# soon-yau/upgpt

Hardware: AMD Instinct MI355X
Metric: 256x256 images/sec, 50-step DDIM, bs=8/GPU; UNet MFMA util % (higher is better)
Workload: dtype f16; 1 GPU; BASELINE configs[1]: bs=8/GPU, 256x256 px (latent 4x32x32), 50-step DDIM eta=0, text-only cond [B,87,768], UNet(bbox.yaml) + VAE decode, EMA weights, no CFG; batch_per_gpu=8, ddim_steps=50, batches_in_flight_per_gpu=4, lane_hw_queues=measured, parallelism=replica-dp1, one all-gather of images per batch

## Files before the change

include/upk.h:

```cpp
#ifndef UPK_H_
#define UPK_H_

#include <stddef.h>
#include <stdint.h>

#ifdef __cplusplus
extern "C" {
#endif

#define UPK_VERSION 100

#define UPK_OK 0
#define UPK_EINVAL (-1)
#define UPK_ESHAPE (-2)
#define UPK_EWORKSPACE (-3)
#define UPK_EHIP (-4)
#define UPK_ENODEV (-5)

typedef struct upk_ctx upk_ctx;
typedef void* upk_stream;

int upk_version(void);
int upk_create(upk_ctx** out, int device);
int upk_destroy(upk_ctx* ctx);
const char* upk_last_error(upk_ctx* ctx);
int upk_set_workspace(upk_ctx* ctx, void* dptr, size_t bytes);
int upk_num_cus(upk_ctx* ctx);

int upk_pack_weight_f16(upk_ctx* ctx, const float* w_oihw, int cout, int cin, int kh, int kw,
                        const int32_t* row_map, int n_rows_packed, const int32_t* col_map,
                        int cin_packed, void* w_packed, upk_stream stream);
size_t upk_packed_weight_bytes(int n_rows_packed, int cin_packed, int kh, int kw);

#define UPK_F_SILU 0x1
#define UPK_F_GEGLU 0x2
#define UPK_F_OUT_F32 0x4
#define UPK_F_OUT_NCHW_F32 0x8
// ... 35 lines not shown
  const void* x4;
  int32_t c3, c4;
  int32_t ld3, ld4;
  const float* gno_gamma;
  const float* gno_beta;
  void* gno_y;
  float gno_eps;
  int32_t gno_silu, gno_ld, gno_skip_y;
  float* ln_rows_out;
  const float* ln_rows_in;
  int32_t ln_rows_slots;
  const void* w_phase;
  int32_t gn_stats_cap;
  const void* pf_next;
  int64_t pf_bytes;
} upk_conv_desc;

int upk_conv2d_nhwc_f16(upk_ctx* ctx, const upk_conv_desc* d, upk_stream stream);

int upk_conv_gn_fused(upk_ctx* ctx, const upk_conv_desc* d, int* mode, int* nblk);
int upk_groupnorm_finalize_f32(upk_ctx* ctx, const float* partials, int nblk, int ld, int batch, int hw, int c,
                               int groups, float* ws, upk_stream stream);
int upk_conv_ln_rows(upk_ctx* ctx, const upk_conv_desc* d, int* slots);

typedef struct upk_mlp_desc {
  const void* x;
  int32_t ldx, m, c, inner;
  const void* w1;
  const float* b1;
  const float* u1;
  float ln_eps;
  int32_t ln_dim;
  const void* w2;
  const float* b2;
  int32_t n_out, n_pad;
  const void* residual;
  int32_t ld_res;
  void* y;
// ... 189 lines not shown
```

upgpt_amd/_lib.py:

```python
import contextlib
import ctypes as C
import os
import threading

import torch
from ._check import require

_HERE = os.path.dirname(os.path.abspath(__file__))
LIB_PATH = os.environ.get("UPK_LIB") or os.path.join(_HERE, "libupk.so")

SYMBOLS = [
    "upk_version", "upk_create", "upk_destroy", "upk_last_error", "upk_set_workspace", "upk_num_cus",
    "upk_pack_weight_f16", "upk_packed_weight_bytes", "upk_conv2d_nhwc_f16", "upk_gemm_f16",
    "upk_conv_autotune", "upk_conv_override", "upk_conv_num_configs", "upk_conv_config_name", "upk_conv_gn_fused",
    "upk_conv_ln_rows",
    "upk_geglu_mlp_f16", "upk_geglu_mlp_supported", "upk_cross_block_f16", "upk_cross_block_supported", "upk_head_block_f16", "upk_head_block_supported",
    "upk_attention_f16", "upk_groupnorm_nhwc_f16", "upk_groupnorm_stats_nhwc_f16", "upk_groupnorm_chunks", "upk_groupnorm_apply_nhwc_f16", "upk_groupnorm_finalize_f32", "upk_groupnorm_ws_bytes",
    "upk_layernorm_f16", "upk_timestep_embed_f16",
    "upk_nchw_f32_to_nhwc_f16", "upk_nhwc_f16_to_nchw_f32", "upk_f32_to_f16", "upk_ddim_step_f32",
    "upk_ddim_step_cfg_f32", "upk_ddim_step_edit_f32", "upk_plms_step_f32", "upk_ddpm_step_f32", "upk_attention_causal_f16", "upk_attention_qproj_f16", "upk_embed_tokens_f16",
    "upk_patchify_nchw_f32_f16", "upk_vit_assemble_f16", "upk_gather_rows_f16",
    "upk_image_finish_u8", "upk_ssim_ws_bytes", "upk_ssim_u8",
    "upk_lpips_input_f16", "upk_relu_pool_nhwc_f16", "upk_lpips_ws_bytes", "upk_lpips_layer_f16",
    "upk_advance_step", "upk_step_autoadvance", "upk_kernel_launches", "upk_graph_begin", "upk_graph_end", "upk_graph_launch", "upk_graph_destroy",
    "upk_prof_enable", "upk_prof_collect",
    "upk_stream_create_cumask", "upk_stream_destroy", "upk_probe_placement", "upk_probe_clock",
]

F_SILU, F_GEGLU, F_OUT_F32, F_OUT_NCHW_F32, F_UPSAMPLE2X, F_PAD_ASYM = 0x1, 0x2, 0x4, 0x8, 0x10, 0x20
DDPM_X0, DDPM_CLIP = 0x1, 0x2
# ... 22 lines not shown
        ("bias", C.c_void_p), ("residual", C.c_void_p), ("ld_res", C.c_int32),
        ("rowvec", C.c_void_p), ("rv_batch_stride", C.c_int32), ("rv_step_stride", C.c_int32),
        ("step", C.c_void_p), ("y", C.c_void_p), ("ldy", C.c_int32),
        ("vt", C.c_void_p), ("vt_from", C.c_int32), ("vt_heads", C.c_int32), ("vt_dhead", C.c_int32),
        ("vt_ld", C.c_int32), ("vt_tokens", C.c_int32), ("flags", C.c_int32),
        ("tune_cfg", C.c_int32), ("tune_splitk", C.c_int32),
        ("ln_colsum", C.c_void_p), ("ln_eps", C.c_float), ("ln_dim", C.c_int32),
        ("gn_stats_ws", C.c_void_p), ("gn_groups", C.c_int32),
        ("x3", C.c_void_p), ("x4", C.c_void_p),
        ("c3", C.c_int32), ("c4", C.c_int32), ("ld3", C.c_int32), ("ld4", C.c_int32),
        ("gno_gamma", C.c_void_p), ("gno_beta", C.c_void_p), ("gno_y", C.c_void_p), ("gno_eps", C.c_float),
        ("gno_silu", C.c_int32), ("gno_ld", C.c_int32), ("gno_skip_y", C.c_int32),
        ("ln_rows_out", C.c_void_p), ("ln_rows_in", C.c_void_p), ("ln_rows_slots", C.c_int32),
        ("w_phase", C.c_void_p), ("gn_stats_cap", C.c_int32),
        ("pf_next", C.c_void_p), ("pf_bytes", C.c_int64),
    ]


class MlpDesc(C.Structure):
    _fields_ = [
        ("x", C.c_void_p), ("ldx", C.c_int32), ("m", C.c_int32), ("c", C.c_int32), ("inner", C.c_int32),
        ("w1", C.c_void_p), ("b1", C.c_void_p), ("u1", C.c_void_p), ("ln_eps", C.c_float), ("ln_dim", C.c_int32),
        ("w2", C.c_void_p), ("b2", C.c_void_p), ("n_out", C.c_int32), ("n_pad", C.c_int32),
        ("residual", C.c_void_p), ("ld_res", C.c_int32), ("y", C.c_void_p), ("ldy", C.c_int32),
        ("gn_stats_ws", C.c_void_p), ("hw", C.c_int32), ("rows_per_wg", C.c_int32),
    ]


class XblockDesc(C.Structure):
    _fields_ = [
        ("a1", C.c_void_p), ("lda", C.c_int32), ("m", C.c_int32), ("c", C.c_int32), ("heads", C.c_int32), ("d", C.c_int32),
# ... 23 lines not shown

def load_library(path=None):
    global _lib
    with _lib_lock:
        if _lib is not None and path is None:
            return _lib
        p = path or LIB_PATH
        if not os.path.exists(p):
            raise RuntimeError(
                "libupk.so not found at %s: build it with `python -m upgpt_amd.build` "
                "(hipcc --offload-arch=gfx950). There is no CPU fallback." % p)
        lib = C.CDLL(p)
        vp, i32, i64, f32 = C.c_void_p, C.c_int, C.c_longlong, C.c_float
        protos = {
            "upk_version": (C.c_int, []),
            "upk_create": (C.c_int, [C.POINTER(vp), i32]),
            "upk_destroy": (C.c_int, [vp]),
            "upk_last_error": (C.c_char_p, [vp]),
            "upk_set_workspace": (C.c_int, [vp, vp, C.c_size_t]),
            "upk_num_cus": (C.c_int, [vp]),
            "upk_pack_weight_f16": (C.c_int, [vp, vp, i32, i32, i32, i32, vp, i32, vp, i32, vp, vp]),
            "upk_packed_weight_bytes": (C.c_size_t, [i32, i32, i32, i32]),
            "upk_conv2d_nhwc_f16": (C.c_int, [vp, C.POINTER(ConvDesc), vp]),
            "upk_gemm_f16": (C.c_int, [vp, vp, i32, i32, i32, vp, i32, i32, vp, vp, i32, vp, i32, i32, vp]),
            "upk_conv_autotune": (C.c_int, [vp, C.POINTER(ConvDesc), vp, i32, C.POINTER(C.c_int), C.POINTER(C.c_int),
                                            C.POINTER(C.c_float), C.POINTER(C.c_float)]),
            "upk_conv_override": (C.c_int, [vp, i32, i32]),
            "upk_conv_num_configs": (C.c_int, []),
            "upk_conv_config_name": (C.c_char_p, [i32]),
            "upk_conv_ln_rows": (C.c_int, [vp, C.POINTER(ConvDesc), C.POINTER(C.c_int)]),
# ... 8 lines not shown
            "upk_attention_causal_f16": (C.c_int, [vp, vp, i32, i64, vp, i32, i64, vp, i32, vp, i32, i64,
                                                   i32, i32, i32, i32, f32, vp]),
            "upk_attention_qproj_f16": (C.c_int, [vp, vp, i32, i64, i32, i32, f32, vp, vp, vp, vp, i32, i64, vp, i32, vp,
                                                  i32, i64, i32, i32, i32, i32, i32, f32, vp]),
            "upk_embed_tokens_f16": (C.c_int, [vp, vp, vp, vp, i32, i32, i32, i32, vp, i32, vp]),
            "upk_gather_rows_f16": (C.c_int, [vp, vp, i32, vp, i32, i32, i32, vp, i32, vp]),
            "upk_patchify_nchw_f32_f16": (C.c_int, [vp, vp, i32, i32, i32, i32, i32, vp, i32, vp]),
            "upk_vit_assemble_f16": (C.c_int, [vp, vp, i32, vp, vp, i32, i32, i32, vp, i32, vp]),
            "upk_groupnorm_nhwc_f16": (C.c_int, [vp, vp, i32, i32, vp, i32, i32, i32, i32, i32, vp, vp,
                                                 f32, i32, vp, i32, vp, vp]),
            "upk_groupnorm_stats_nhwc_f16": (C.c_int, [vp, vp, i32, i32, vp, i32, i32, i32, i32, i32, vp, vp]),
            "upk_groupnorm_chunks": (C.c_int, [i32]),
            "upk_groupnorm_apply_nhwc_f16": (C.c_int, [vp, vp, i32, i32, vp, i32, i32, i32, i32, i32, vp, vp,
                                                       f32, i32, vp, i32, vp, i32, i32, i32, vp, i32, i32, vp]),
            "upk_conv_gn_fused": (C.c_int, [vp, C.POINTER(ConvDesc), C.POINTER(C.c_int), C.POINTER(C.c_int)]),
            "upk_groupnorm_finalize_f32": (C.c_int, [vp, vp, i32, i32, i32, i32, i32, i32, vp, vp]),
            "upk_groupnorm_ws_bytes": (C.c_size_t, [i32, i32]),
            "upk_layernorm_f16": (C.c_int, [vp, vp, i32, i32, i32, vp, vp, f32, vp, i32, vp]),
            "upk_timestep_embed_f16": (C.c_int, [vp, vp, i32, i32, f32, vp, i32, vp]),
            "upk_nchw_f32_to_nhwc_f16": (C.c_int, [vp, vp, i32, i32, i32, vp, i32, i32, i32, f32, vp]),
            "upk_nhwc_f16_to_nchw_f32": (C.c_int, [vp, vp, i32, i32, i32, i32, vp, vp]),
            "upk_f32_to_f16": (C.c_int, [vp, vp, i32, i32, vp, i32, vp]),
            "upk_ddim_step_f32": (C.c_int, [vp, vp, vp, vp, vp, vp, vp, vp, i32, i32, i32, i32, vp]),
            "upk_ddim_step_cfg_f32": (C.c_int, [vp, vp, vp, vp, vp, vp, vp, vp, i32, i32, i32, i32, f32, vp]),
            "upk_ddim_step_edit_f32": (C.c_int, [vp, vp, vp, vp, vp, vp, vp, i32, vp, vp, vp, vp, i32, i32, i32, i32, f32,
                                                 i32, vp]),
            "upk_plms_step_f32": (C.c_int, [vp, vp, vp, vp, vp, vp, vp, vp, i32, i32, i32, i32, f32, i32, vp]),
            "upk_ddpm_step_f32": (C.c_int, [vp, vp, vp, vp, vp, vp, vp, vp, vp, vp, vp, i32, i32, i32, i32, i32, vp]),
            "upk_image_finish_u8": (C.c_int, [vp, vp, i32, i32, i32, i32, i64, i32, i32, i32, i32, vp, i64, i32, i64, i32,
                                              C.POINTER(C.c_float), vp]),
# ... 10 lines not shown
            "upk_graph_end": (C.c_int, [vp, vp, C.POINTER(vp)]),
            "upk_graph_launch": (C.c_int, [vp, vp, vp]),
            "upk_graph_destroy": (C.c_int, [vp, vp]),
            "upk_prof_enable": (C.c_int, [vp, i32]),
            "upk_prof_collect": (C.c_int, [vp, C.POINTER(C.c_double), C.POINTER(C.c_longlong)]),
            "upk_stream_create_cumask": (C.c_int, [vp, C.POINTER(C.c_uint32), i32, C.POINTER(vp)]),
            "upk_stream_destroy": (C.c_int, [vp, vp]),
            "upk_probe_placement": (C.c_int, [vp, vp, i32, i32, vp]),
            "upk_probe_clock": (C.c_int, [vp, vp, i64, vp]),
        }
        require(sorted(protos) == sorted(SYMBOLS), "ctypes prototypes and SYMBOLS differ", RuntimeError)
        for name, (res, args) in protos.items():
            fn = getattr(lib, name)
            fn.restype = res
            fn.argtypes = args
        if path is None:
            _lib = lib
        return lib


def _ptr(t):
    if t is None:
        return None
    if isinstance(t, int):
        return t
    return t.data_ptr()


class Context:

# ... 61 lines not shown
        self._chk(self.lib.upk_embed_tokens_f16(self.h, _ptr(ids), _ptr(tok), _ptr(pos), rows, seq, dim, vocab, _ptr(out),
                                                ld, self._s()))

    def gather_rows(self, x, ldx, idx, n, n_src, dim, y, ldy):
        self._chk(self.lib.upk_gather_rows_f16(self.h, _ptr(x), ldx, _ptr(idx), n, n_src, dim, _ptr(y), ldy, self._s()))

    def groupnorm(self, x1, c1, ld1, x2, c2, ld2, batch, hw, groups, gamma, beta, eps, silu, y, ldy, ws):
        self._chk(self.lib.upk_groupnorm_nhwc_f16(self.h, _ptr(x1), c1, ld1, _ptr(x2), c2, ld2, batch, hw, groups,
                                                  _ptr(gamma), _ptr(beta), eps, int(silu), _ptr(y), ldy, _ptr(ws),
                                                  self._s()))

    def conv_gn_fused(self, desc):
        f, n = C.c_int(0), C.c_int(0)
        self._chk(self.lib.upk_conv_gn_fused(self.h, C.byref(desc), C.byref(f), C.byref(n)))
        return f.value, n.value

    def gn_stats_floats(self, batch, n_pad, cap=32):
        return batch * max(32, cap) * 2 * max(n_pad, 32)

    def groupnorm_ws_bytes(self, batch, hw):
        return self.lib.upk_groupnorm_ws_bytes(batch, hw)

    def layernorm(self, x, ldx, rows, d, gamma, beta, eps, y, ldy):
        self._chk(self.lib.upk_layernorm_f16(self.h, _ptr(x), ldx, rows, d, _ptr(gamma), _ptr(beta), eps,
                                             _ptr(y), ldy, self._s()))

    def timestep_embed(self, t, n, dim, max_period, out, ld_out):
        self._chk(self.lib.upk_timestep_embed_f16(self.h, _ptr(t), n, dim, max_period, _ptr(out), ld_out, self._s()))

    def nchw_to_nhwc(self, x, batch, c, hw, y, ldy, c_off=0, zero_pad_to=0, scale=1.0):
# ... 205 lines not shown
```

upgpt_amd/csrc/igemm.hip:

```cpp
#include "igemm_common.h"

namespace {
using namespace upkd;


template <int MI, int NI, int WM, int WN, int KS>
__global__ __launch_bounds__(WM* WN * 64) void igemm_kernel(const IgemmArgs a) {
  constexpr int BM = MI * 16 * WM;
  constexpr int BN = NI * 16 * WN;
  constexpr int NT = WM * WN * 64;
  constexpr int A_IT = (BM * 4 + NT - 1) / NT;
  constexpr int B_IT = (BN * 4 + NT - 1) / NT;
  constexpr int A_TILE = BM * 32;
  constexpr int B_TILE = BN * 32;
  constexpr int A_STAGE = KS * A_TILE;
  constexpr int B_STAGE = KS * B_TILE;

  __shared__ __attribute__((aligned(16))) f16 smem[2 * (A_STAGE + B_STAGE)];
  f16* sA = smem;
  f16* sB = smem + 2 * A_STAGE;

  const int tid = threadIdx.x;
  const int lane = tid & 63;
  const int wave = tid >> 6;
// ... 178 lines not shown
    return;
  }
  if (a.partial) {
    slab_t* slab = (slab_t*)a.partial + ((long)zs * (a.ph_on ? 4 : 1) + ph) * a.M * a.npad;
#pragma unroll
    for (int i = 0; i < MI; ++i) {
      const int m = mw + i * 16 + lc;
      if (m >= a.M) continue;
      const unsigned roff = (unsigned)m * (unsigned)a.npad;
#pragma unroll
      for (int j = 0; j < NI; ++j) {
        const int n = nw + j * 16 + lg * 4;
        if (n < a.npad && !ABL_ON(ABL_NOSLAB)) slab_store(slab + roff + n, acc[i][j]);
      }
    }
    return;
  }
  if (a.lnr_in) Epi::lnr_fix<MI, NI>(a, mw, nw, lc, lg, acc);
  Epi::tile<MI, NI, WM, WN>(a, m0, mw, nw, lc, lg, acc, wm, wn, (float*)smem, a.M);
}


template <int P>
__device__ __forceinline__ void wait_vmcnt() {
  asm volatile("s_waitcnt vmcnt(%0)" ::"n"(P) : "memory");
}

template <int MI, int NI, int WM, int WN, int KS, int NBUF, bool APP = false, bool LNF = false, int LW = 4>
__global__ __launch_bounds__(256 + LW * 64) void igemm_ws_kernel(const IgemmArgs a) {
  static_assert(WM * WN == 4 || WM * WN == 1, "4 consumer waves");
// ... 343 lines not shown
    if ABL_ON(ABL_NOEPI) return;
    auto frag_sum = [&](int f) {
      f32x4 v = *(const f32x4*)(red + ((0 * NF + f) * 64 + lane) * 4);
#pragma unroll
      for (int w = 1; w < 4; ++w) v += *(const f32x4*)(red + ((w * NF + f) * 64 + lane) * 4);
      return v;
    };
    slab_t* slab = a.partial ? (slab_t*)a.partial + ((long)zs * (a.ph_on ? 4 : 1) + ph) * a.M * a.npad : nullptr;
    if (slab) {
      for (int f = wave; f < NF; f += EW) {
        const int i = f / NI, j = f - i * NI;
        const int m = m0 + i * 16 + lc;
        const int n = n0 + j * 16 + lg * 4;
        if (n < a.npad && m < a.M && !ABL_ON(ABL_NOSLAB)) slab_store(slab + (unsigned)m * (unsigned)a.npad + n, frag_sum(f));
      }
      return;
    }
    constexpr int FW = (NF + EW - 1) / EW;
    if (Epi::plain(a)) {
      const Epi::Plain P(a);
      Epi::Plain::Row rows[FW];
      f32x4 bvs[FW], rvs[FW];
      f16x4 rrs[FW];
#pragma unroll
      for (int q = 0; q < FW; ++q) {
        const int f = wave + EW * q;
        const int i = f / NI, j = f - i * NI;
        const int n = n0 + j * 16 + lg * 4;
        rows[q] = P.row(a, f < NF ? m0 + i * 16 + lc : a.M, a.M);
        bvs[q] = P.bias4(a, n);
// ... 147 lines not shown
    return;
  }
  if (a.partial) {
    slab_t* slab = (slab_t*)a.partial + ((long)zs * (a.ph_on ? 4 : 1) + ph) * a.M * a.npad;
#pragma unroll
    for (int i = 0; i < MI; ++i) {
      const int m = mw + i * 16 + lc;
      if (m >= a.M) continue;
      const unsigned roff = (unsigned)m * (unsigned)a.npad;
#pragma unroll
      for (int j = 0; j < NI; ++j) {
        const int n = nw + j * 16 + lg * 4;
        if (n < a.npad && !ABL_ON(ABL_NOSLAB)) slab_store(slab + roff + n, acc[i][j]);
      }
    }
    return;
  }
  if constexpr (SHARE) {
    if (Epi::plain(a) && !a.lnr_out) {
      float* hand = (float*)((char*)smem + HAND_OFF) + wave * (MI * NJ1) * 256;
      f32x4 acc1[MI][NJ0];
#pragma unroll
      for (int i = 0; i < MI; ++i)
#pragma unroll
        for (int j = 0; j < NI; ++j) {
          if (j < NJ0) acc1[i][j] = acc[i][j];
          else *(f32x4*)(hand + ((i * NJ1 + (j - NJ0)) * 64 + lane) * 4) = acc[i][j];
        }
      asm volatile("s_waitcnt lgkmcnt(0)" ::: "memory");
      __builtin_amdgcn_s_barrier();
// ... 13 lines not shown
  if (wave == 0) {
    asm volatile("s_waitcnt vmcnt(0)" ::: "memory");
    STAMP(4);
  }
#endif
#undef STAMP
}

__global__ __launch_bounds__(256) void igemm_reduce_kernel(const IgemmArgs a, int splitk) {
  const int nq = a.npad >> 2;
  const long idx = (long)blockIdx.x * 256 + threadIdx.x;
  const long total = (long)a.M * nq;
  if (idx >= total) return;
  const int m = (int)(idx / nq);
  const int n = (int)(idx - (long)m * nq) * 4;
  const long slab = (long)a.M * a.npad * (a.ph_on ? 4 : 1);
  const slab_t* p = (const slab_t*)a.partial + ((long)ph_id(a) * a.M + m) * a.npad + n;
  f32x4 v = {0, 0, 0, 0}, g = {0, 0, 0, 0};
  const f32x4 z4 = {0.f, 0.f, 0.f, 0.f};
  if (a.flags & UPK_F_GEGLU) {
    if (n & 32) return;
    for (int z = 0; z < splitk; ++z) {
      v += slab_load4(p + z * slab);
      g += slab_load4(p + z * slab + 32);
    }
  } else {
    for (int z0 = 0; z0 < splitk; z0 += 4) {
      f32x4 t[4];
#pragma unroll
      for (int u = 0; u < 4; ++u) t[u] = z0 + u < splitk ? slab_load4(p + (long)(z0 + u) * slab) : z4;
#pragma unroll
      for (int u = 0; u < 4; ++u) v += t[u];
    }
  }
  IgemmArgs b = a;
  b.partial = nullptr;
  const RowCtx rc = Epi::row(b, m, b.M);
  Epi::store(b, rc, n, v, g, Epi::bias4(b, n), Epi::bias4(b, (a.flags & UPK_F_GEGLU) ? n + 32 : a.npad),
             Epi::fetch(b, rc, n));
}

struct GnApply {
  const float* gamma;
  const float* beta;
  f16* yn;
  float eps;
  int ldn, silu, skip_y, cpg, hw;
};

template <int V>
struct VecIO {
  static __device__ __forceinline__ void ldf(const float* p, bool on, float (&o)[V]) {
    if constexpr (V == 4) {
      const f32x4 w = on ? *(const f32x4*)p : (f32x4){0.f, 0.f, 0.f, 0.f};
// ... 308 lines not shown
extern "C" int upk_conv_num_configs(void) { return kNumCfgs + astat_num_configs() + bt_num_configs(); }
extern "C" const char* upk_conv_config_name(int cfg) {
  if (cfg >= kNumCfgs + astat_num_configs()) return bt_config_name(cfg - kNumCfgs - astat_num_configs());
  if (cfg >= kNumCfgs) return astat_config_name(cfg - kNumCfgs);
  return (cfg >= 0 && cfg < kNumCfgs) ? kCfgs[cfg].name : "?";
}
extern "C" int upk_conv_override(upk_ctx* ctx, int cfg, int splitk) {
  if (!ctx) return UPK_EINVAL;
  if (cfg >= upk_conv_num_configs()) return upk_fail(ctx, UPK_EINVAL, "conv_override: configuration %d of %d", cfg, upk_conv_num_configs());
  ctx->cfg_override = cfg;
  ctx->splitk_override = splitk;
  return UPK_OK;
}

static int conv_impl(upk_ctx* ctx, const upk_conv_desc* d, upk_stream stream_, bool launch, int* gn_fused,
                     int* gn_nblk = nullptr, int* lnr_slots = nullptr) {
  if (lnr_slots) *lnr_slots = 0;
  if (!ctx || !d) return UPK_EINVAL;
  hipStream_t stream = (hipStream_t)stream_;
  if (!d->x1 || !d->w_packed || !d->y) return upk_fail(ctx, UPK_EINVAL, "conv: null x1/w/y");
  if (d->c1 <= 0 || (d->c1 & 31) || (d->c2 & 31) || d->c2 < 0)
    return upk_fail(ctx, UPK_ESHAPE, "conv: channels must be multiples of 32 (c1=%d c2=%d)", d->c1, d->c2);
  if (d->c2 > 0 && !d->x2) return upk_fail(ctx, UPK_EINVAL, "conv: c2>0 but x2 null");
  if (d->ksize != 1 && d->ksize != 3) return upk_fail(ctx, UPK_ESHAPE, "conv: ksize %d", d->ksize);
  if (d->stride != 1 && d->stride != 2) return upk_fail(ctx, UPK_ESHAPE, "conv: stride %d", d->stride);
  if ((d->ld1 & 7) || (d->c2 && (d->ld2 & 7)) || (d->n_pad & 15) || d->n_pad <= 0)
    return upk_fail(ctx, UPK_EINVAL, "conv: leading dims must be multiples of 8, n_pad of 16");
  const int flags = d->flags;
  const bool geglu = flags & UPK_F_GEGLU;
  if (geglu && (d->n_pad & 63)) return upk_fail(ctx, UPK_ESHAPE, "conv: GEGLU needs n_pad %% 64 == 0");
  if (!(flags & UPK_F_OUT_NCHW_F32) && (d->ldy & 3)) return upk_fail(ctx, UPK_EINVAL, "conv: ldy %% 4");
  if (d->residual && (d->ld_res & 3)) return upk_fail(ctx, UPK_EINVAL, "conv: ld_res %% 4");
// ... 133 lines not shown
    best = want_cfg;
    best_sk = sk;
  }
  const bool is_as = want_cfg >= kNumCfgs && !is_bt;
  if (is_as) {
    if (!astat_plan(ctx, a, want_cfg - kNumCfgs, want_sk, &aspl) || (want_sk > 1 && want_sk > aspl.npass))
      return upk_fail(ctx, UPK_ESHAPE, "conv: A-stationary configuration %s (passes per workgroup %d) does not fit this launch",
                      astat_config_name(want_cfg - kNumCfgs), want_sk);
    best = want_cfg;
    best_sk = 1;
  }
  for (int c = 0; c < kNumCfgs && !is_as && !is_bt; ++c) {
    if (want_cfg >= 0 && c != want_cfg) continue;
    if (a.ln_u && !a.lnr_in && !kCfgs[c].fn_ln) continue;
    if (a.x3 && !kCfgs[c].fn_app) continue;
    for (int sk : sk_cands) {
      if (want_sk > 0 && sk != want_sk) continue;
      if (a.ln_u && sk > 1) continue;
      if (sk > 1 && (slab * sk > ctx->ws_bytes || a.nchunks / sk < 4)) continue;
      const double t = estimate(kCfgs[c], a.M * nph, a.npad, a.nchunks, sk, ctx->num_cus, geglu);
      if (t < best_t) {
        best_t = t;
        best = c;
        best_sk = sk;
      }
    }
  }
  if (want_cfg < 0 && want_sk <= 1 && bt_able && Epi::plain(a) && best >= 0 && best_sk == 1) {
    for (int c = 0; c < bt_num_configs(); ++c) {
      int bm, bn, occ, mi, ni, wn;
      bt_tile(c, &bm, &bn, &occ, &mi, &ni, &wn);
      if (geglu && ((ni * 16) % 64 != 0)) continue;
// ... 52 lines not shown
  const bool gn_cp = !a.ph_on && d->gn_stats_ws && zdim == 1 && Epi::plain(a) && d->gn_groups > 0 &&
                     d->gn_groups <= UPK_GN_GROUPS_MAX && a.n_out % d->gn_groups == 0 && a.n_out <= 2048 &&
                     hw_out % BM == 0 && hw_out / BM <= (d->gn_stats_cap > UPK_GN_MAX_CHUNKS ? d->gn_stats_cap : UPK_GN_MAX_CHUNKS);
  if (gn_cp) {
    a.gn_cp = d->gn_stats_ws;
    a.gn_nblk = hw_out / BM;
    a.gn_hw = hw_out;
  }
  if (d->ln_rows_out && !a.ph_on && zdim == 1 && Epi::plain(a) && !gn_cp && (is_as || is_bt || c.wm * c.wn > 1 || c.nbuf > 0)) {
    const int slots = is_as ? (aspl.npass == 1 ? cdiv(a.npad, astat_config_ni(best - kNumCfgs) * 16) : 99)
                            : a.tiles_n * (is_bt ? bt_wn : c.wn);
    if (slots <= 8) {
      a.lnr_out = d->ln_rows_out;
      if (lnr_slots) *lnr_slots = slots;
    }
  }
  if (gn_fused) *gn_fused = gn_apply ? 3 : (gn_fuse ? 1 : (gn_cp ? 2 : 0));
  if (gn_nblk) *gn_nblk = gn_cp ? a.gn_nblk : 0;
  if (!launch) return UPK_OK;

#ifdef UPK_TIMELINE
  {
    static int launch_no = 0;
    static const char* tgt = getenv("UPK_TL_TARGET");
    if (tgt) {
      a.flags &= ~ABL_TIMELINE;
      if (launch_no == atoi(tgt)) {
        a.flags |= ABL_TIMELINE;
        fprintf(stderr, "[timeline] launch %d: M=%d npad=%d nchunks=%d ks=%d cfg=%s(%d) splitk=%d flags=%x res=%d rowvec=%d\n", launch_no,
                a.M, a.npad, a.nchunks, a.ks, upk_conv_config_name(best), best, zdim, flags, a.res != nullptr, a.rowvec != nullptr);
// ... 65 lines not shown
      hipLaunchKernelGGL((igemm_reduce_gnapply_kernel<4, 8>), gg, dim3(256), 0, stream, a, zdim, g);
    else if (ga_v == 2)
      hipLaunchKernelGGL((igemm_reduce_gnapply_kernel<2, 8>), gg, dim3(256), 0, stream, a, zdim, g);
    else
      hipLaunchKernelGGL((igemm_reduce_gnapply_kernel<1, 32>), gg, dim3(256), 0, stream, a, zdim, g);
    rc = upk_check_launch(ctx, "igemm_reduce_gnapply");
  } else if (zdim > 1 && gn_fuse) {
    GnFuse gf;
    gf.ws = d->gn_stats_ws;
    gf.groups = d->gn_groups;
    gf.cpg = a.n_out / d->gn_groups;
    gf.hw = a.Ho * a.Wo;
    upk_gn_chunking(gf.hw, &gf.nchunks, &gf.pix_per_chunk);
    hipLaunchKernelGGL(igemm_reduce_gn_kernel, dim3(gf.nchunks, a.B), dim3(256), 0, stream, a, zdim, gf);
    rc = upk_check_launch(ctx, "igemm_reduce_gn");
  } else if (zdim > 1) {
    const long total = (long)a.M * (a.npad / 4);
    hipLaunchKernelGGL(igemm_reduce_kernel, dim3((unsigned)((total + 255) / 256), nph), dim3(256), 0, stream, a, zdim);
    rc = upk_check_launch(ctx, "igemm_reduce");
  }
  return rc;
}

extern "C" int upk_conv2d_nhwc_f16(upk_ctx* ctx, const upk_conv_desc* d, upk_stream stream) {
  return conv_impl(ctx, d, stream, true, nullptr);
}

extern "C" int upk_conv_ln_rows(upk_ctx* ctx, const upk_conv_desc* d, int* slots) {
  if (!slots) return UPK_EINVAL;
  return conv_impl(ctx, d, nullptr, false, nullptr, nullptr, slots);
}

extern "C" int upk_conv_gn_fused(upk_ctx* ctx, const upk_conv_desc* d, int* mode, int* nblk) {
  if (!mode || !nblk) return UPK_EINVAL;
  *mode = 0;
  *nblk = 0;
  return conv_impl(ctx, d, nullptr, false, mode, nblk);
}

constexpr float kGnStatsLaunchUs = 5.0f;

extern "C" int upk_conv_autotune(upk_ctx* ctx, const upk_conv_desc* d, upk_stream stream_, int reps, int* best_cfg,
                                 int* best_splitk, float* best_us, float* default_us) {
  if (!ctx || !d || !best_cfg || !best_splitk) return UPK_EINVAL;
  if (ctx->prof_on) return upk_fail(ctx, UPK_EINVAL, "autotune with profiling enabled");
// ... 101 lines not shown
```

upgpt_amd/csrc/igemm_common.h:

```cpp
#pragma once
#include <stdlib.h>

#include "common.h"

namespace upkd {

enum {
  ABL_NOEPI = 0x10000,
  ABL_NOGLOAD = 0x20000,
  ABL_NOLDSW = 0x40000,
  ABL_NOMFMA = 0x80000,
  ABL_EMPTY = 0x100000,
  ABL_TIMELINE = 0x200000,
  ABL_NOSTORE = 0x400000,
  ABL_NOGNP = 0x800000,
  ABL_NOEPILD = 0x1000000,
  ABL_NOSLAB = 0x2000000,
  ABL_NOA = 0x4000000,
  ABL_NOB = 0x8000000,
};
#if defined(UPK_DEV) || defined(UPK_TIMELINE)
#define ABL_ON(f) ((a.flags & (f)) != 0)
#else
#define ABL_ON(f) (false)
// ... 39 lines not shown
  int chunks_per_split;
  int tiles_m, tiles_n;
  int flags;
  int tile_rows;
  float* lnr_out;
  const float* lnr_in;
  int lnr_slots;
  int ph_on;
  int ph_wstride;
  int sh_hw, sh_w;
  int xm_pm, xm_pn, xm_mi, xm_nj, xm_z;
  int as_ppw, as_npass;
  const char* pf;
  int pf_lines;
  int pf_self;
};

#ifdef UPK_SLAB_F32
typedef float slab_t;
typedef f32x4 slab4;
#else
typedef f16 slab_t;
typedef f16x4 slab4;
#endif
__device__ __forceinline__ void slab_store(slab_t* p, f32x4 v) {
#ifdef UPK_SLAB_F32
  asm volatile("global_store_dwordx4 %0, %1, off sc1" ::"v"(p), "v"(v) : "memory");
#else
  const f16x4 h = {(f16)__builtin_amdgcn_fmed3f(v[0], -65504.f, 65504.f), (f16)__builtin_amdgcn_fmed3f(v[1], -65504.f, 65504.f),
                   (f16)__builtin_amdgcn_fmed3f(v[2], -65504.f, 65504.f), (f16)__builtin_amdgcn_fmed3f(v[3], -65504.f, 65504.f)};
  asm volatile("global_store_dwordx2 %0, %1, off sc1" ::"v"(p), "v"(h) : "memory");
#endif
}
__device__ __forceinline__ f32x4 slab_load4(const slab_t* p) {
  const slab4 v = *(const slab4*)p;
  return (f32x4){(float)v[0], (float)v[1], (float)v[2], (float)v[3]};
}

__device__ __forceinline__ bool tile_map(const IgemmArgs& a, int& tm, int& tn, int& zs) {
  if (a.xm_pm == 0) {
    const int tile = blockIdx.x;
    tn = tile / a.tiles_m;
    tm = tile - tn * a.tiles_m;
    zs = blockIdx.z;
    return true;
  }
  const int w = blockIdx.x;
  const int xcd = w & 7, l = w >> 3;
  const int xi = xcd / a.xm_pn, xj = xcd - xi * a.xm_pn;
  const int ul = l / a.xm_mi, tl = l - ul * a.xm_mi;
  tm = xi * a.xm_mi + tl;
// ... 434 lines not shown
        if (geglu) {
          if constexpr (NI % 4 == 0) {
            if ((j & 2) == 0) store(a, rc, n, acc[i][j], acc[i][j + 2 < NI ? j + 2 : j], bias4(a, n), bias4(a, n + 32),
                                    fetch(a, rc, n));
          }
        } else {
          const f32x4 b = bias4(a, n);
          store(a, rc, n, acc[i][j], acc[i][j], b, b, fetch(a, rc, n));
        }
      }
    }
  }
};


struct AsPlan {
  int bm, pw, npass, ppw, tiles_m, tiles_n, lds_bytes;
};
int astat_num_configs();
const char* astat_config_name(int c);
int astat_config_ni(int c);
bool astat_plan(const upk_ctx* ctx, const IgemmArgs& a, int c, int ppw_req, AsPlan* pl);
int astat_launch(upk_ctx* ctx, IgemmArgs& a, int c, const AsPlan& pl, dim3 grid, hipStream_t stream);

int bt_num_configs();
const char* bt_config_name(int c);
void bt_tile(int c, int* bm, int* bn, int* occ, int* mi, int* ni, int* wn);
bool bt_full_epilogue(int c);
int bt_launch(upk_ctx* ctx, const IgemmArgs& a, int c, dim3 grid, hipStream_t stream);

// ... 4 lines not shown
```

upgpt_amd/csrc/misc.hip:

```cpp
#include <stdarg.h>

#include "common.h"

extern "C" int upk_version(void) { return UPK_VERSION; }

extern "C" int upk_create(upk_ctx** out, int device) {
  if (!out) return UPK_EINVAL;
  *out = nullptr;
  int n = 0;
  if (hipGetDeviceCount(&n) != hipSuccess || n <= 0 || device < 0 || device >= n) return UPK_ENODEV;
  hipDeviceProp_t prop;
  if (hipGetDeviceProperties(&prop, device) != hipSuccess) return UPK_EHIP;
  if (strncmp(prop.gcnArchName, "gfx950", 6) != 0) return UPK_ENODEV;
  upk_ctx* c = new upk_ctx();
  c->device = device;
  c->num_cus = prop.multiProcessorCount;
  c->err[0] = 0;
  c->ws = nullptr;
  c->ws_bytes = 0;
  c->zero_page = nullptr;
  c->tune_flush = nullptr;
  c->step_done = nullptr;
  c->n_kernels = 0;
  {
// ... 699 lines not shown
```

upgpt_amd/emitter.py:

```python
import ctypes as C
import os

import torch

from . import _lib as L
from . import knobs as K
from ._check import require
from .packing import PW, Packer, _rup, head_pad
from .tuning import TUNE_CACHE, TUNE_CACHE_LANES


class Act:
    __slots__ = ("t", "B", "H", "W", "C", "gn_src", "ln_src")

    def __init__(self, t, B, H, W, C):
        self.t, self.B, self.H, self.W, self.C = t, B, H, W, C
        self.ln_src = None
        self.gn_src = None

    @property
    def ld(self):
        return self.t.shape[-1]

    @property
# ... 72 lines not shown
            ent = lookup(overlay, key) if overlay is not None else None
            if ent is None:
                ent = lookup(cache, key)
            if ent is None and tune_missing:
                cfg, sk, best_us, dflt_us = self.ctx.conv_autotune(d, reps or int(os.environ.get("UPGPT_TUNE_REPS", "5")))
                ent = cache.put(key, cfg, sk, best_us, dflt_us)
                tuned += 1
            elif ent is not None:
                hits += 1
            else:
                missing += 1
            if ent is not None:
                d.tune_cfg, d.tune_splitk = int(ent[0]) + 1, int(ent[1])
        if tuned and cache.dirty and os.environ.get("UPGPT_TUNE_SAVE"):
            cache.save(os.environ["UPGPT_TUNE_SAVE"])
        return hits, tuned, missing

    def link_weight_prefetch(self, prog, wrap=True):
        mode = K.WEIGHT_PREFETCH
        if mode == "0" or (mode == "auto" and L.concurrency() > 1):
            return 0
        ds = [d for d in prog.meta if d is not None and getattr(d, "_w_bytes", 0)]
        n = 0
        ahead = max(1, K.WEIGHT_PREFETCH_AHEAD)
        for i, d in enumerate(ds):
            j = i + ahead
            nxt = ds[j] if j < len(ds) else (ds[j % len(ds)] if wrap and len(ds) > ahead else None)
            if nxt is None or nxt.w_packed == d.w_packed:
                continue
            d.pf_next, d.pf_bytes = nxt.w_packed, min(nxt._w_bytes, K.WEIGHT_PREFETCH_MAX)
            n += 1
# ... 455 lines not shown
```

upgpt_amd/knobs.py:

```python
import os

VAE_GN_BYPRODUCT = os.environ.get("UPGPT_VAE_GN_BYPRODUCT", "0")
VAE_GN_MINM = int(os.environ.get("UPGPT_VAE_GN_MINM", "131072"))


def vae_gn_byproduct(M):
    return VAE_GN_BYPRODUCT == "1" or (VAE_GN_BYPRODUCT == "auto" and M >= VAE_GN_MINM)
UPS_PHASES = os.environ.get("UPGPT_UPS_PHASES", "1") == "1"
LN_ROWS = os.environ.get("UPGPT_LN_ROWS", "1") == "1"
QPROJ_FUSE = os.environ.get("UPGPT_QPROJ_FUSE", "1") == "1"
GN_REDUCE_APPLY = os.environ.get("UPGPT_GN_REDUCE_APPLY", "1") == "1"
MLP_FUSE = os.environ.get("UPGPT_MLP_FUSE", "auto")
MLP_ROWS = int(os.environ.get("UPGPT_MLP_ROWS", "0"))
XBLOCK = os.environ.get("UPGPT_XBLOCK", "auto")
XB_ROWS = int(os.environ.get("UPGPT_XB_ROWS", "0"))
HBLOCK = os.environ.get("UPGPT_HBLOCK", "auto")
HBLOCK_GN = os.environ.get("UPGPT_HBLOCK_GN", "1") == "1"
WEIGHT_PREFETCH = os.environ.get("UPGPT_WEIGHT_PREFETCH", "auto")
WEIGHT_PREFETCH_AHEAD = int(os.environ.get("UPGPT_WEIGHT_PREFETCH_AHEAD", "1"))
WEIGHT_PREFETCH_MAX = int(os.environ.get("UPGPT_WEIGHT_PREFETCH_MAX", str(32 << 20)))
LN_LAUNCH_US = 5.0
```

Measured before the change: 94.60 images/s.

## Fuse split-K reduction into igemm via per-tile atomic tickets

```diff
diff --git a/include/upk.h b/include/upk.h
--- a/include/upk.h
+++ b/include/upk.h
@@ -9,6 +9,7 @@
 #endif
 
 #define UPK_VERSION 100
+#define UPK_DESC_ABI 2
 
 #define UPK_OK 0
 #define UPK_EINVAL (-1)
@@ -21,6 +22,8 @@
 typedef void* upk_stream;
 
 int upk_version(void);
+int upk_desc_abi(void);
+size_t upk_conv_desc_bytes(void);
 int upk_create(upk_ctx** out, int device);
 int upk_destroy(upk_ctx* ctx);
 const char* upk_last_error(upk_ctx* ctx);
@@ -86,6 +89,8 @@
   int32_t gn_stats_cap;
   const void* pf_next;
   int64_t pf_bytes;
+  uint32_t* sk_tickets;
+  int32_t sk_ticket_cap;
 } upk_conv_desc;
 
 int upk_conv2d_nhwc_f16(upk_ctx* ctx, const upk_conv_desc* d, upk_stream stream);
@@ -94,6 +99,7 @@
 int upk_groupnorm_finalize_f32(upk_ctx* ctx, const float* partials, int nblk, int ld, int batch, int hw, int c,
                                int groups, float* ws, upk_stream stream);
 int upk_conv_ln_rows(upk_ctx* ctx, const upk_conv_desc* d, int* slots);
+int upk_conv_splitk_tickets(upk_ctx* ctx, const upk_conv_desc* d, int* n);
 
 typedef struct upk_mlp_desc {
   const void* x;
diff --git a/upgpt_amd/_lib.py b/upgpt_amd/_lib.py
--- a/upgpt_amd/_lib.py
+++ b/upgpt_amd/_lib.py
@@ -10,10 +10,10 @@
 LIB_PATH = os.environ.get("UPK_LIB") or os.path.join(_HERE, "libupk.so")
 
 SYMBOLS = [
-    "upk_version", "upk_create", "upk_destroy", "upk_last_error", "upk_set_workspace", "upk_num_cus",
+    "upk_version", "upk_desc_abi", "upk_conv_desc_bytes", "upk_create", "upk_destroy", "upk_last_error", "upk_set_workspace", "upk_num_cus",
     "upk_pack_weight_f16", "upk_packed_weight_bytes", "upk_conv2d_nhwc_f16", "upk_gemm_f16",
     "upk_conv_autotune", "upk_conv_override", "upk_conv_num_configs", "upk_conv_config_name", "upk_conv_gn_fused",
-    "upk_conv_ln_rows",
+    "upk_conv_ln_rows", "upk_conv_splitk_tickets",
     "upk_geglu_mlp_f16", "upk_geglu_mlp_supported", "upk_cross_block_f16", "upk_cross_block_supported", "upk_head_block_f16", "upk_head_block_supported",
     "upk_attention_f16", "upk_groupnorm_nhwc_f16", "upk_groupnorm_stats_nhwc_f16", "upk_groupnorm_chunks", "upk_groupnorm_apply_nhwc_f16", "upk_groupnorm_finalize_f32", "upk_groupnorm_ws_bytes",
     "upk_layernorm_f16", "upk_timestep_embed_f16",
@@ -66,7 +66,11 @@
         ("ln_rows_out", C.c_void_p), ("ln_rows_in", C.c_void_p), ("ln_rows_slots", C.c_int32),
         ("w_phase", C.c_void_p), ("gn_stats_cap", C.c_int32),
         ("pf_next", C.c_void_p), ("pf_bytes", C.c_int64),
+        ("sk_tickets", C.c_void_p), ("sk_ticket_cap", C.c_int32),
     ]
+
+
+DESC_ABI = 2
 
 
 class MlpDesc(C.Structure):
@@ -120,6 +124,8 @@
         vp, i32, i64, f32 = C.c_void_p, C.c_int, C.c_longlong, C.c_float
         protos = {
             "upk_version": (C.c_int, []),
+            "upk_desc_abi": (C.c_int, []),
+            "upk_conv_desc_bytes": (C.c_size_t, []),
             "upk_create": (C.c_int, [C.POINTER(vp), i32]),
             "upk_destroy": (C.c_int, [vp]),
             "upk_last_error": (C.c_char_p, [vp]),
@@ -158,6 +164,7 @@
             "upk_groupnorm_apply_nhwc_f16": (C.c_int, [vp, vp, i32, i32, vp, i32, i32, i32, i32, i32, vp, vp,
                                                        f32, i32, vp, i32, vp, i32, i32, i32, vp, i32, i32, vp]),
             "upk_conv_gn_fused": (C.c_int, [vp, C.POINTER(ConvDesc), C.POINTER(C.c_int), C.POINTER(C.c_int)]),
+            "upk_conv_splitk_tickets": (C.c_int, [vp, C.POINTER(ConvDesc), C.POINTER(C.c_int)]),
             "upk_groupnorm_finalize_f32": (C.c_int, [vp, vp, i32, i32, i32, i32, i32, i32, vp, vp]),
             "upk_groupnorm_ws_bytes": (C.c_size_t, [i32, i32]),
             "upk_layernorm_f16": (C.c_int, [vp, vp, i32, i32, i32, vp, vp, f32, vp, i32, vp]),
@@ -198,6 +205,10 @@
             fn = getattr(lib, name)
             fn.restype = res
             fn.argtypes = args
+        require(lib.upk_desc_abi() == DESC_ABI and lib.upk_conv_desc_bytes() == C.sizeof(ConvDesc),
+                "libupk.so was built from another include/upk.h (descriptor ABI %d, upk_conv_desc of %d bytes; this "
+                "binding: %d, %d): rebuild it" % (lib.upk_desc_abi(), lib.upk_conv_desc_bytes(), DESC_ABI,
+                                                   C.sizeof(ConvDesc)), RuntimeError)
         if path is None:
             _lib = lib
         return lib
@@ -289,6 +300,11 @@
         f, n = C.c_int(0), C.c_int(0)
         self._chk(self.lib.upk_conv_gn_fused(self.h, C.byref(desc), C.byref(f), C.byref(n)))
         return f.value, n.value
+
+    def conv_splitk_tickets(self, desc):
+        n = C.c_int(0)
+        self._chk(self.lib.upk_conv_splitk_tickets(self.h, C.byref(desc), C.byref(n)))
+        return n.value
 
     def gn_stats_floats(self, batch, n_pad, cap=32):
         return batch * max(32, cap) * 2 * max(n_pad, 32)
diff --git a/upgpt_amd/csrc/igemm.hip b/upgpt_amd/csrc/igemm.hip
--- a/upgpt_amd/csrc/igemm.hip
+++ b/upgpt_amd/csrc/igemm.hip
@@ -216,6 +216,7 @@
         if (n < a.npad && !ABL_ON(ABL_NOSLAB)) slab_store(slab + roff + n, acc[i][j]);
       }
     }
+    if (a.tickets) splitk_finish<BM, BN, NT>(a, tm, tn, tid, (unsigned*)smem);
     return;
   }
   if (a.lnr_in) Epi::lnr_fix<MI, NI>(a, mw, nw, lc, lg, acc);
@@ -589,6 +590,7 @@
         const int n = n0 + j * 16 + lg * 4;
         if (n < a.npad && m < a.M && !ABL_ON(ABL_NOSLAB)) slab_store(slab + (unsigned)m * (unsigned)a.npad + n, frag_sum(f));
       }
+      if (a.tickets) splitk_finish<BM, BN, EW * 64>(a, tm, tn, tid, (unsigned*)smem);
       return;
     }
     constexpr int FW = (NF + EW - 1) / EW;
@@ -766,6 +768,7 @@
         if (n < a.npad && !ABL_ON(ABL_NOSLAB)) slab_store(slab + roff + n, acc[i][j]);
       }
     }
+    if (a.tickets) splitk_finish<BM, BN, 256>(a, tm, tn, tid, (unsigned*)smem);
     return;
   }
   if constexpr (SHARE) {
@@ -809,30 +812,7 @@
   if (idx >= total) return;
   const int m = (int)(idx / nq);
   const int n = (int)(idx - (long)m * nq) * 4;
-  const long slab = (long)a.M * a.npad * (a.ph_on ? 4 : 1);
-  const slab_t* p = (const slab_t*)a.partial + ((long)ph_id(a) * a.M + m) * a.npad + n;
-  f32x4 v = {0, 0, 0, 0}, g = {0, 0, 0, 0};
-  const f32x4 z4 = {0.f, 0.f, 0.f, 0.f};
-  if (a.flags & UPK_F_GEGLU) {
-    if (n & 32) return;
-    for (int z = 0; z < splitk; ++z) {
-      v += slab_load4(p + z * slab);
-      g += slab_load4(p + z * slab + 32);
-    }
-  } else {
-    for (int z0 = 0; z0 < splitk; z0 += 4) {
-      f32x4 t[4];
-#pragma unroll
-      for (int u = 0; u < 4; ++u) t[u] = z0 + u < splitk ? slab_load4(p + (long)(z0 + u) * slab) : z4;
-#pragma unroll
-      for (int u = 0; u < 4; ++u) v += t[u];
-    }
-  }
-  IgemmArgs b = a;
-  b.partial = nullptr;
-  const RowCtx rc = Epi::row(b, m, b.M);
-  Epi::store(b, rc, n, v, g, Epi::bias4(b, n), Epi::bias4(b, (a.flags & UPK_F_GEGLU) ? n + 32 : a.npad),
-             Epi::fetch(b, rc, n));
+  splitk_reduce_store<false>(a, splitk, m, n);
 }
 
 struct GnApply {
@@ -1171,8 +1151,9 @@
 }
 
 static int conv_impl(upk_ctx* ctx, const upk_conv_desc* d, upk_stream stream_, bool launch, int* gn_fused,
-                     int* gn_nblk = nullptr, int* lnr_slots = nullptr) {
+                     int* gn_nblk = nullptr, int* lnr_slots = nullptr, int* sk_tickets = nullptr) {
   if (lnr_slots) *lnr_slots = 0;
+  if (sk_tickets) *sk_tickets = 0;
   if (!ctx || !d) return UPK_EINVAL;
   hipStream_t stream = (hipStream_t)stream_;
   if (!d->x1 || !d->w_packed || !d->y) return upk_fail(ctx, UPK_EINVAL, "conv: null x1/w/y");
@@ -1336,8 +1317,9 @@
     if (want_cfg >= 0 && c != want_cfg) continue;
     if (a.ln_u && !a.lnr_in && !kCfgs[c].fn_ln) continue;
     if (a.x3 && !kCfgs[c].fn_app) continue;
-    for (int sk : sk_cands) {
-      if (want_sk > 0 && sk != want_sk) continue;
+    for (int sk0 : sk_cands) {
+      if (want_sk > 0 && sk0 != sk_cands[0]) continue;
+      const int sk = want_sk > 0 ? want_sk : sk0;
       if (a.ln_u && sk > 1) continue;
       if (sk > 1 && (slab * sk > ctx->ws_bytes || a.nchunks / sk < 4)) continue;
       const double t = estimate(kCfgs[c], a.M * nph, a.npad, a.nchunks, sk, ctx->num_cus, geglu);
@@ -1420,6 +1402,12 @@
       a.lnr_out = d->ln_rows_out;
       if (lnr_slots) *lnr_slots = slots;
     }
+  }
+  const int sk_need = (zdim > 1 && !gn_apply && !gn_fuse && !is_as && !is_bt) ? a.tiles_m * a.tiles_n * nph : 0;
+  if (sk_tickets) *sk_tickets = sk_need;
+  if (sk_need && d->sk_tickets) {
+    if (((uintptr_t)d->sk_tickets) & 3) return upk_fail(ctx, UPK_EINVAL, "conv: sk_tickets must be 4-byte aligned");
+    if (d->sk_ticket_cap >= sk_need) a.tickets = d->sk_tickets;
   }
   if (gn_fused) *gn_fused = gn_apply ? 3 : (gn_fuse ? 1 : (gn_cp ? 2 : 0));
   if (gn_nblk) *gn_nblk = gn_cp ? a.gn_nblk : 0;
@@ -1515,7 +1503,7 @@
     upk_gn_chunking(gf.hw, &gf.nchunks, &gf.pix_per_chunk);
     hipLaunchKernelGGL(igemm_reduce_gn_kernel, dim3(gf.nchunks, a.B), dim3(256), 0, stream, a, zdim, gf);
     rc = upk_check_launch(ctx, "igemm_reduce_gn");
-  } else if (zdim > 1) {
+  } else if (zdim > 1 && !a.tickets) {
     const long total = (long)a.M * (a.npad / 4);
     hipLaunchKernelGGL(igemm_reduce_kernel, dim3((unsigned)((total + 255) / 256), nph), dim3(256), 0, stream, a, zdim);
     rc = upk_check_launch(ctx, "igemm_reduce");
@@ -1530,6 +1518,11 @@
 extern "C" int upk_conv_ln_rows(upk_ctx* ctx, const upk_conv_desc* d, int* slots) {
   if (!slots) return UPK_EINVAL;
   return conv_impl(ctx, d, nullptr, false, nullptr, nullptr, slots);
+}
+
+extern "C" int upk_conv_splitk_tickets(upk_ctx* ctx, const upk_conv_desc* d, int* n) {
+  if (!n) return UPK_EINVAL;
+  return conv_impl(ctx, d, nullptr, false, nullptr, nullptr, nullptr, n);
 }
 
 extern "C" int upk_conv_gn_fused(upk_ctx* ctx, const upk_conv_desc* d, int* mode, int* nblk) {
diff --git a/upgpt_amd/csrc/igemm_common.h b/upgpt_amd/csrc/igemm_common.h
--- a/upgpt_amd/csrc/igemm_common.h
+++ b/upgpt_amd/csrc/igemm_common.h
@@ -77,6 +77,7 @@
   const char* pf;
   int pf_lines;
   int pf_self;
+  unsigned* tickets;
 };
 
 #ifdef UPK_SLAB_F32
@@ -98,6 +99,18 @@
 __device__ __forceinline__ f32x4 slab_load4(const slab_t* p) {
   const slab4 v = *(const slab4*)p;
   return (f32x4){(float)v[0], (float)v[1], (float)v[2], (float)v[3]};
+}
+__device__ __forceinline__ f32x4 slab_load4_dev(const slab_t* p) {
+  typedef __attribute__((address_space(1))) unsigned long long gu64;
+#ifdef UPK_SLAB_F32
+  const unsigned long long lo = __hip_atomic_load((gu64*)p, __ATOMIC_RELAXED, __HIP_MEMORY_SCOPE_AGENT);
+  const unsigned long long hi = __hip_atomic_load((gu64*)p + 1, __ATOMIC_RELAXED, __HIP_MEMORY_SCOPE_AGENT);
+  const f32x2 a = __builtin_bit_cast(f32x2, lo), b = __builtin_bit_cast(f32x2, hi);
+  return (f32x4){a[0], a[1], b[0], b[1]};
+#else
+  const slab4 v = __builtin_bit_cast(slab4, __hip_atomic_load((gu64*)p, __ATOMIC_RELAXED, __HIP_MEMORY_SCOPE_AGENT));
+  return (f32x4){(float)v[0], (float)v[1], (float)v[2], (float)v[3]};
+#endif
 }
 
 __device__ __forceinline__ bool tile_map(const IgemmArgs& a, int& tm, int& tn, int& zs) {
@@ -562,6 +575,59 @@
 };
 
 
+template <bool DEV>
+__device__ __forceinline__ void splitk_reduce_store(const IgemmArgs& a, int splitk, int m, int n) {
+  const long slab = (long)a.M * a.npad * (a.ph_on ? 4 : 1);
+  const slab_t* p = (const slab_t*)a.partial + ((long)ph_id(a) * a.M + m) * a.npad + n;
+  f32x4 v = {0, 0, 0, 0}, g = {0, 0, 0, 0};
+  const f32x4 z4 = {0.f, 0.f, 0.f, 0.f};
+  if (a.flags & UPK_F_GEGLU) {
+    if (n & 32) return;
+    for (int z = 0; z < splitk; ++z) {
+      v += DEV ? slab_load4_dev(p + z * slab) : slab_load4(p + z * slab);
+      g += DEV ? slab_load4_dev(p + z * slab + 32) : slab_load4(p + z * slab + 32);
+    }
+  } else {
+    for (int z0 = 0; z0 < splitk; z0 += 4) {
+      f32x4 t[4];
+#pragma unroll
+      for (int u = 0; u < 4; ++u)
+        t[u] = z0 + u < splitk ? (DEV ? slab_load4_dev(p + (long)(z0 + u) * slab) : slab_load4(p + (long)(z0 + u) * slab)) : z4;
+#pragma unroll
+      for (int u = 0; u < 4; ++u) v += t[u];
+    }
+  }
+  IgemmArgs b = a;
+  b.partial = nullptr;
+  const RowCtx rc = Epi::row(b, m, b.M);
+  Epi::store(b, rc, n, v, g, Epi::bias4(b, n), Epi::bias4(b, (a.flags & UPK_F_GEGLU) ? n + 32 : a.npad),
+             Epi::fetch(b, rc, n));
+}
+
+template <int BM, int BN, int NT>
+__device__ __forceinline__ void splitk_finish(const IgemmArgs& a, int tm, int tn, int t, unsigned* flag) {
+  asm volatile("s_waitcnt vmcnt(0)" ::: "memory");
+  __syncthreads();
+  if (t == 0) {
+    typedef __attribute__((address_space(1))) unsigned gu32;
+    gu32* tk = (gu32*)a.tickets + ((long)ph_id(a) * a.tiles_n + tn) * a.tiles_m + tm;
+    const unsigned got = __hip_atomic_fetch_add(tk, 1u, __ATOMIC_RELAXED, __HIP_MEMORY_SCOPE_AGENT);
+    const bool last = got == (unsigned)(a.xm_z - 1);
+    if (last) __hip_atomic_store(tk, 0u, __ATOMIC_RELAXED, __HIP_MEMORY_SCOPE_AGENT);
+    *flag = last ? 1u : 0u;
+  }
+  __syncthreads();
+  if (*flag == 0u) return;
+  __builtin_amdgcn_fence(__ATOMIC_ACQUIRE, "wavefront");
+  constexpr int NQ = BN / 4;
+  const int m0 = tm * BM, n0 = tn * BN;
+  for (int idx = t; idx < BM * NQ; idx += NT) {
+    const int r = idx / NQ;
+    const int m = m0 + r, n = n0 + (idx - r * NQ) * 4;
+    if (m < a.M && n < a.npad) splitk_reduce_store<true>(a, a.xm_z, m, n);
+  }
+}
+
 struct AsPlan {
   int bm, pw, npass, ppw, tiles_m, tiles_n, lds_bytes;
 };
diff --git a/upgpt_amd/csrc/misc.hip b/upgpt_amd/csrc/misc.hip
--- a/upgpt_amd/csrc/misc.hip
+++ b/upgpt_amd/csrc/misc.hip
@@ -3,6 +3,8 @@
 #include "common.h"
 
 extern "C" int upk_version(void) { return UPK_VERSION; }
+extern "C" int upk_desc_abi(void) { return UPK_DESC_ABI; }
+extern "C" size_t upk_conv_desc_bytes(void) { return sizeof(upk_conv_desc); }
 
 extern "C" int upk_create(upk_ctx** out, int device) {
   if (!out) return UPK_EINVAL;
diff --git a/upgpt_amd/emitter.py b/upgpt_amd/emitter.py
--- a/upgpt_amd/emitter.py
+++ b/upgpt_amd/emitter.py
@@ -110,7 +110,20 @@
                 d.tune_cfg, d.tune_splitk = int(ent[0]) + 1, int(ent[1])
         if tuned and cache.dirty and os.environ.get("UPGPT_TUNE_SAVE"):
             cache.save(os.environ["UPGPT_TUNE_SAVE"])
+        self.n_splitk_fused = self.arm_splitk_finish()
         return hits, tuned, missing
+
+    def arm_splitk_finish(self):
+        n = 0
+        for d, _ in self.convs:
+            need = self.ctx.conv_splitk_tickets(d) if K.SPLITK_FUSE else 0
+            if need:
+                t = self.alloc(need, dtype=torch.int32, zero=True)
+                d.sk_tickets, d.sk_ticket_cap = t.data_ptr(), need
+                n += 1
+            else:
+                d.sk_tickets, d.sk_ticket_cap = None, 0
+        return n
 
     def link_weight_prefetch(self, prog, wrap=True):
         mode = K.WEIGHT_PREFETCH
diff --git a/upgpt_amd/knobs.py b/upgpt_amd/knobs.py
--- a/upgpt_amd/knobs.py
+++ b/upgpt_amd/knobs.py
@@ -19,4 +19,5 @@
 WEIGHT_PREFETCH = os.environ.get("UPGPT_WEIGHT_PREFETCH", "auto")
 WEIGHT_PREFETCH_AHEAD = int(os.environ.get("UPGPT_WEIGHT_PREFETCH_AHEAD", "1"))
 WEIGHT_PREFETCH_MAX = int(os.environ.get("UPGPT_WEIGHT_PREFETCH_MAX", str(32 << 20)))
+SPLITK_FUSE = os.environ.get("UPGPT_SPLITK_FUSE", "1") == "1"
 LN_LAUNCH_US = 5.0
```

Result: slower. 91.16 images/s (-3.6%).
